# cuevhv/PMT_learning_for_semantic_segmentation_and_disparity

Measured on AMD Instinct MI355X. Metric: stereo-pairs/sec (train fwd+bwd) 512x256, higher is better.
Workload: dtype bf16; 1 GPU; minidsnetExt (densenet121, 1dcorr, aspp 0; the live PyTorch form of baseline_SDnet*) train step fwd+loss(CE+CE+Lovasz+L1)+bwd+Adam, 512x256 (WxH), batch 8 per GPU, hipGraph; global_batch=8, parallelism=dp1, world_size=1

## Files before the change

### include/sdhip.h

```cpp
#ifndef SDHIP_H_
#define SDHIP_H_

#include <stdint.h>

#ifdef __cplusplus
extern "C" {
#endif

#define SDHIP_F32 0
#define SDHIP_BF16 1

#define SDHIP_OK 0
#define SDHIP_ERR_ARG (-1)
#define SDHIP_ERR_LAUNCH (-2)
#define SDHIP_ERR_UNSUPPORTED (-3)

#define SDHIP_ACT_HSWISH 5
#define SDHIP_ACT_HSIGMOID 6

int sdhip_abi_version(void);
const char* sdhip_last_error(void);
void sdhip_diag_reload(void);
int sdhip_abort_capture(void* stream);
int sdhip_graph_node_counts(void* graph, int* counts);
// ... 12 lines not shown
int sdhip_conv_pack_weights(const float* src, void* dst, int M, int K, int T,
                            long stride_m, long stride_k, int flip, int dtype, void* stream);
int sdhip_conv_unpack_wgrad(const float* acc, float* grad, int M, int K, int T,
                            long stride_m, long stride_k, int flip, int accumulate, int dtype, void* stream);

int sdhip_conv2d_fwd(const void* x, const void* wpacked, void* y,
                     const float* bias, const float* in_scale, const float* in_shift,
                     double* stats, int stats_ld, int stats_nrep,
                     int B, int H, int W, int Cin, int ldx,
                     int Ho, int Wo, int Cout, int ldy,
                     int kh, int kw, int stride, int dil, int pad_t, int pad_l,
                     int D, int Do, int kd, int sd, int pad_d,
                     int in_relu, int groups, int act, int accumulate,
                     int dtype, void* stream);

int sdhip_conv2d_fwd_bnpro(const void* x, const void* wpacked, void* y, double* out_stats, int out_stats_ld, int out_stats_nrep,
                           double* in_stats, int in_stats_ld, int in_stats_nrep,
                           const double* pend_stats, int pend_ld, int pend_nrep, int pend_c0, int pend_n,
                           const float* gamma, const float* beta,
                           float* running_mean, float* running_var, float* scale_out, float* shift_out, float* mean_out,
                           float* invstd_out, double count, float eps, float momentum,
                           int B, int H, int W, int Cin, int ldx, int Ho, int Wo, int Cout, int ldy,
                           int kh, int kw, int pad_t, int pad_l, int groups, int dtype, void* stream);

int sdhip_conv2d_fwd_add(const void* x, const void* wpacked, void* y, const void* addend, int ldadd,
                         int B, int H, int W, int Cin, int ldx, int Ho, int Wo, int Cout, int ldy,
                         int kh, int kw, int pad_t, int pad_l, int dtype, void* stream);

int sdhip_conv2d_fwd_bnbwd(const void* x, const void* wpacked, void* y, double* sums, int sums_ld, int sums_nrep,
                           const void* u, int ldu, const float* scale, const float* shift, const void* addend, int ldadd,
                           int B, int H, int W, int Cin, int ldx, int Ho, int Wo, int Cout, int ldy,
                           int kh, int kw, int dil, int pad_t, int pad_l, int groups, int mode, int dtype, void* stream);

int sdhip_conv2d_fwd_phase(const void* x, const void* wpacked, void* y, double* stats, int stats_ld, int stats_nrep,
                           int B, int H, int W, int Cin, int ldx, int Cout, int ldy, int kh, int kw,
                           int D, int kd, int groups, int off_d, int off_h, int off_w, int dtype, void* stream);
int sdhip_conv2d_wgrad(const void* x, const void* dy, float* dw_packed, float* dbias,
                       const float* in_scale, const float* in_shift,
                       int B, int H, int W, int Cin, int ldx,
                       int Ho, int Wo, int Cout, int lddy,
                       int kh, int kw, int stride, int dil, int pad_t, int pad_l,
                       int D, int Do, int kd, int sd, int pad_d,
                       int in_relu, int groups, int prezeroed, int dtype, void* stream);
typedef struct SdhipWgradItem {
  const void* x; const void* dy; float* dw_packed; float* dbias; const float* in_scale; const float* in_shift;
  int B, H, W, Cin, ldx, Ho, Wo, Cout, lddy, kh, kw, stride, dil, pad_t, pad_l, D, Do, kd, sd, pad_d, in_relu, groups;
// ... 199 lines not shown
```

### pmt_learning_for_semantic_segmentation_and_disparity_amd/csrc/conv_fast.h

```cpp
#pragma once
#include "conv_common.h"

namespace {

struct FastArgs {
  const void* x; const void* wp; void* y;
  const float* bias; const float* in_scale; const float* in_shift; double* stats;
  int B, H, W, Ho, Wo, kh, kw, stride, dil, pad_t, pad_l;
  int D, Do, kd, sd, pad_d;
  int Cin, ldx, Cout, Mpad, ldy;
  int in_relu, bpg, act, accumulate;
  unsigned magic_iwp, magic_tw;
  int tiles_w, ntg;
  int tg, stats_ld, nrep, tail, dma;
  long rep_stride;
  int omul, ooz, ooy, oox;
  const void* bx; const float* bsc; const float* bsh; int ldbx;
  const void* res; int ldres;
  int bx_mode, bx_groups;
  const double* pin_stats; int pin_ld, pin_nrep, pin_groups, pin_off, pin_cs;
  const float* pin_gamma; const float* pin_beta;
  float* pin_scale; float* pin_shift; float* pin_mean; float* pin_invstd; float* pin_rmean; float* pin_rvar;
  float pin_eps, pin_momentum; double pin_count;
  const double* pend_stats; double* pin_fold; int pend_ld, pend_nrep, pend_c0, pend_n;
// ... 11 lines not shown
#pragma clang diagnostic pop
__device__ __forceinline__ unsigned lds_addr(const void* p) {
  return (unsigned)(size_t)(const __attribute__((address_space(3))) unsigned char*)p;
}

template <int CTRL> __device__ __forceinline__ float dpp_add(float v) {
  return v + __builtin_bit_cast(float, __builtin_amdgcn_update_dpp(0, __builtin_bit_cast(int, v), CTRL, 0xf, 0xf, true));
}
__device__ __forceinline__ float row16_sum(float v) {
  v = dpp_add<0xB1>(v);
  v = dpp_add<0x4E>(v);
  v = dpp_add<0x141>(v);
  return dpp_add<0x140>(v);
}

template <int KS> struct LdsRow;
template <> struct LdsRow<2> {
  static __device__ __forceinline__ int off(int row, int c) { return row * 128 + ((c ^ (row & 6)) << 4); }
};
template <> struct LdsRow<1> {
  static __device__ __forceinline__ int off(int row, int c) { return row * 64 + ((c ^ ((row >> 1) & 2)) << 4); }
};

template <typename T, int TH, int TW, int BN, int KS, bool DMA, bool BX = false>
__global__ __launch_bounds__(256) void conv_fast_kernel(const FastArgs p) {
  constexpr int V = Chunk<T>::N;
  constexpr int CK = 8 * V;
  constexpr int CKS = 4 * KS * V;
  constexpr int RB = 64 * KS;
  constexpr int SH = KS + 1;
  constexpr int CH = 4 * KS;
  constexpr int TWT = TW / 16, NPT = TH * TWT, NT_PIX = NPT / 4, NT_CO = BN / 16;
  constexpr bool PF = (TH * TW <= 64);
  constexpr int HPF = (DMA && KS == 1) ? 6 : 5;
  static_assert(NPT % 4 == 0 && NT_PIX >= 1, "every wave needs at least one 16-pixel MFMA tile");
  extern __shared__ __attribute__((aligned(16))) unsigned char smem[];

  const int tid = threadIdx.x, lane = tid & 63, wave = tid >> 6;
  const int l15 = lane & 15, lg = lane >> 4;
  const int s = p.stride, d = p.dil;
  const int tiles_w = p.tiles_w;
  const int ty = fast_div(blockIdx.x, tiles_w, p.magic_tw);
  const int oh0 = ty * TH, ow0 = (blockIdx.x - ty * tiles_w) * TW;
  const int n0 = blockIdx.y * BN;
  const int b = p.Do == 1 ? (int)blockIdx.z : (int)blockIdx.z / p.Do, dz = blockIdx.z - b * p.Do;
  const int grp = b < p.bpg ? 0 : b / p.bpg;
  const int IH = (TH - 1) * s + (p.kh - 1) * d + 1, IW = (TW - 1) * s + (p.kw - 1) * d + 1;
  const int IWp = (IW + 7) & ~7;
  const int ih0 = oh0 * s - p.pad_t, iw0 = ow0 * s - p.pad_l;
  const int Tn = p.kh * p.kw;
  const int nq = KS == 2 ? (p.Cin + CK - 1) / CK : 1;
  const int nqq = p.kd * nq;
  const int halo_bytes = ((IH * IWp + (256 >> SH) - 1) & ~((256 >> SH) - 1)) * RB;
  const int wbuf_bytes = ((p.tg * BN + (256 >> SH) - 1) & ~((256 >> SH) - 1)) * RB;
  unsigned char* const halo0 = smem;
  unsigned char* const wl0 = smem + halo_bytes * ((PF && nqq > 1) ? 2 : 1);

  f32x4 acc[NT_CO][NT_PIX];
#pragma unroll
  for (int mi = 0; mi < NT_CO; ++mi)
#pragma unroll
    for (int ni = 0; ni < NT_PIX; ++ni) acc[mi][ni] = f32x4{0.f, 0.f, 0.f, 0.f};

  const T* const xb0 = (const T*)p.x + (long)b * p.D * p.H * p.W * p.ldx;
  const T* const wpk = (const T*)p.wp;
  const int ntg = p.ntg;

  const int pt0 = wave * NT_PIX;
  const int prow0 = ((pt0 / TWT) * s) * IWp + ((pt0 % TWT) * 16 + l15) * s;
  int pdelta[NT_PIX];
#pragma unroll
  for (int ni = 0; ni < NT_PIX; ++ni) {
    const int pt = pt0 + ni;
    pdelta[ni] = (((pt / TWT) - (pt0 / TWT)) * s * IWp + ((pt % TWT) - (pt0 % TWT)) * 16 * s) * RB;
  }
  const int lg4 = lg << 4;
  const int a_base = LdsRow<KS>::off(l15, lg);

  constexpr int RPR = 256 >> SH;
  const int rsub = tid >> SH;
  const int c_l = (tid & (CH - 1)) ^ (KS == 2 ? (rsub & 6) : ((rsub >> 1) & 2));
  const int tid16 = tid * 16;
  const unsigned wave_lds = __builtin_amdgcn_readfirstlane(lds_addr(smem) + wave * 1024);
  const unsigned magic_iwp = p.magic_iwp;
  constexpr bool dma = DMA;
  float* const ptab_sc = reinterpret_cast<float*>(smem + (DMA ? 0 : p.pin_off));
  float* const ptab_sh = ptab_sc + (DMA ? 0 : p.pin_cs);
  const bool has_pro = p.in_scale != nullptr || (!DMA && p.pin_stats != nullptr);
  const int h_rows = IH * IWp;
  const int h_rounds = (h_rows + RPR - 1) / RPR;
  int h_src[HPF];
  if constexpr (PF) {
#pragma unroll
    for (int j = 0; j < HPF; ++j) {
      const int row = rsub + j * RPR;
      const int ih = fast_div(row, IWp, magic_iwp), iw = row - ih * IWp;
      const int gh = ih0 + ih, gw = iw0 + iw;
      h_src[j] = (row < h_rows && iw < IW && gh >= 0 && gh < p.H && gw >= 0 && gw < p.W) ? (gh * p.W + gw) * p.ldx + c_l * V : -1;
    }
  }
  const int mvalid = min(BN, p.Mpad - n0);

  u32x4 rh[HPF];
  const bool flat = p.kd == 1;
  auto chunk_of = [&](int qq) { return flat ? qq : qq % nq; };
  auto slice_of = [&](int qq) { return flat ? dz * p.sd - p.pad_d : dz * p.sd + qq / nq - p.pad_d; };

  auto mask_tail = [&](u32x4 raw, int ch0) -> u32x4 {
    const int nv = p.Cin - ch0;
    if (nv < V) {
      float f[V];
      Chunk<T>::unpack(raw, f);
#pragma unroll
      for (int e = 0; e < V; ++e) f[e] = e < nv ? f[e] : 0.f;
      raw = Chunk<T>::pack(f);
    }
    return raw;
  };
  float psc[V], psf[V];
  auto prologue_load = [&](int ch0) {
    if (ch0 < p.Cin) {
      if constexpr (!DMA) {
        if (p.pin_stats) {
#pragma unroll
          for (int e = 0; e < V; ++e) { psc[e] = ptab_sc[ch0 + e]; psf[e] = ptab_sh[ch0 + e]; }
          return;
// ... 28 lines not shown
#pragma unroll
    for (int j = 0; j < HPF; ++j) {
      if (j < h_rounds) {
        const T* src = (ok && h_src[j] >= 0) ? xb + h_src[j] : (const T*)sdhip_zero16;
        if constexpr (dma) glds16(src, (unsigned)(dst - smem) + j * 4096 + wave_lds);
        else rh[j] = *reinterpret_cast<const u32x4*>(src);
      }
    }
  };
  auto halo_commit = [&](int qq, unsigned char* dst) {
    const int ch0 = chunk_of(qq) * CKS + c_l * V;
    const int din = slice_of(qq);
    const bool ok = din >= 0 && din < p.D && ch0 < p.Cin;
    if (has_pro) prologue_load(ch0);
#pragma unroll
    for (int j = 0; j < HPF; ++j) {
      if (j < h_rounds) {
        u32x4 raw = rh[j];
        if (ok && h_src[j] >= 0) {
          if (p.tail) raw = mask_tail(raw, ch0);
          if (has_pro) raw = prologue(raw);
        }
        *reinterpret_cast<u32x4*>(dst + j * 4096 + tid16) = raw;
      }
    }
  };
  auto halo_sync_stage = [&](int qq, unsigned char* dst) {
    const int ch0 = chunk_of(qq) * CKS + c_l * V;
    const int din = slice_of(qq);
    const bool ok = din >= 0 && din < p.D && ch0 < p.Cin;
    const T* xb = xb0 + (long)din * p.H * p.W * p.ldx + ch0;
    auto src_of = [&](int j) -> const T* {
      const int row = rsub + j * RPR;
      const int ih = fast_div(row, IWp, magic_iwp), iw = row - ih * IWp;
      const int gh = ih0 + ih, gw = iw0 + iw;
      const bool in = ok && iw < IW && gh >= 0 && gh < p.H && gw >= 0 && gw < p.W;
      return in ? xb + (gh * p.W + gw) * p.ldx : (const T*)sdhip_zero16;
    };
    if constexpr (dma) {
      for (int j = 0; j < h_rounds; ++j) glds16(src_of(j), (unsigned)(dst - smem) + j * 4096 + wave_lds);
    } else {
      if (has_pro) prologue_load(ch0);
      for (int j0 = 0; j0 < h_rounds; j0 += 4) {
        u32x4 raw[4];
        bool in[4];
#pragma unroll
        for (int j = 0; j < 4; ++j) {
          if (j0 + j < h_rounds) {
            const T* src = src_of(j0 + j);
            in[j] = src != (const T*)sdhip_zero16;
            raw[j] = *reinterpret_cast<const u32x4*>(src);
          }
        }
#pragma unroll
        for (int j = 0; j < 4; ++j) {
          if (j0 + j < h_rounds) {
            if (in[j] && p.tail) raw[j] = mask_tail(raw[j], ch0);
            if (in[j] && has_pro) raw[j] = prologue(raw[j]);
            *reinterpret_cast<u32x4*>(dst + (j0 + j) * 4096 + tid16) = raw[j];
          }
        }
      }
    }
  };
  constexpr int RPT = BN >= RPR ? BN / RPR : 1;
  constexpr int TPR = BN >= RPR ? 1 : RPR / BN;
  auto w_issue = [&](int qq, int t0, unsigned char* dst) {
    const int nt = min(p.tg, Tn - t0);
    const T* base = wpk + ((long)(qq * Tn + t0) * p.Mpad + n0) * CK + c_l * V;
    unsigned lds = (unsigned)(dst - smem) + wave_lds;
    if constexpr (BN >= RPR) {
      for (int tl = 0; tl < nt; ++tl) {
#pragma unroll
        for (int r = 0; r < RPT; ++r) {
          const int m = min(r * RPR + rsub, mvalid - 1);
          glds16(base + (tl * p.Mpad + m) * CK, lds);
          lds += 4096;
        }
      }
    } else {
      const int m = min(rsub % BN, mvalid - 1);
      for (int t = 0; t < nt; t += TPR) {
        const int tl = min(t + rsub / BN, nt - 1);
        glds16(base + (tl * p.Mpad + m) * CK, lds);
        lds += 4096;
      }
    }
  };

  int kwi = 0, tap_off = 0;
  const int tap_row_step = d * IWp - p.kw * d;
  auto compute = [&](int t0, const unsigned char* halo, const unsigned char* wl) {
    const int nt = min(p.tg, Tn - t0);
    const int n = nt * KS;
    u32x4 af[2][NT_CO], bf[2][NT_PIX];
    int b_addr = 0, a_addr = 0;
    auto next_tap = [&](int tl) {
      const int row = prow0 + tap_off;
      if constexpr (KS == 2) b_addr = row * RB + (lg4 ^ ((row & 6) << 4));
      else b_addr = row * RB + (lg4 ^ (((row >> 1) & 2) << 4));
      a_addr = a_base + tl * (BN * RB);
      tap_off += d;
      if (++kwi == p.kw) { kwi = 0; tap_off += tap_row_step; }
    };
    auto load = [&](int set, int ks) {
      const unsigned char* ab = wl + (a_addr ^ (ks << 6));
      const unsigned char* bb = halo + (b_addr ^ (ks << 6));
#pragma unroll
      for (int mi = 0; mi < NT_CO; ++mi) af[set][mi] = *reinterpret_cast<const u32x4*>(ab + mi * (16 * RB));
#pragma unroll
      for (int ni = 0; ni < NT_PIX; ++ni) bf[set][ni] = *reinterpret_cast<const u32x4*>(bb + pdelta[ni]);
    };
    auto mma = [&](int set) {
#pragma unroll
      for (int mi = 0; mi < NT_CO; ++mi)
#pragma unroll
        for (int ni = 0; ni < NT_PIX; ++ni) Mma<T>::run(acc[mi][ni], af[set][mi], bf[set][ni]);
    };
    if constexpr (KS == 2) {
      next_tap(0);
      load(0, 0);
      for (int tl = 0; tl < nt; ++tl) {
        load(1, 1);
        mma(0);
        if (tl + 1 < nt) { next_tap(tl + 1); load(0, 0); }
        mma(1);
      }
    } else {
      next_tap(0);
      load(0, 0);
      for (int u = 0; u < n; u += 2) {
        if (u + 1 < n) { next_tap(u + 1); load(1, 0); }
        mma(0);
        if (u + 2 < n) { next_tap(u + 2); load(0, 0); }
        if (u + 1 < n) mma(1);
      }
    }
  };

  w_issue(0, 0, wl0);
  if constexpr (PF) halo_issue(0, halo0);
  if constexpr (!DMA) {
    if (p.pin_stats) {
      const int G = p.pin_groups;
      auto sums_of = [&](int g, int c, double& a1, double& a2) {
        a1 = 0.; a2 = 0.;
        const int cp = c - p.pend_c0;
        if (cp >= 0 && cp < p.pend_n) {
          for (int r = 0; r < p.pend_nrep; ++r) {
            const double* Sr = p.pend_stats + (long)r * G * 2 * p.pend_ld;
            a1 += Sr[((long)g * 2 + 0) * p.pend_ld + cp];
            a2 += Sr[((long)g * 2 + 1) * p.pend_ld + cp];
          }
        } else {
          for (int r = 0; r < p.pin_nrep; ++r) {
            const double* Sr = p.pin_stats + (long)r * G * 2 * p.pin_ld;
            a1 += Sr[((long)g * 2 + 0) * p.pin_ld + c];
            a2 += Sr[((long)g * 2 + 1) * p.pin_ld + c];
          }
        }
      };
      for (int c = tid; c < p.Cin; c += 256) {
        double a1, a2;
        sums_of(grp, c, a1, a2);
        const double mu = a1 / p.pin_count;
        double var = a2 / p.pin_count - mu * mu;
// ... 11 lines not shown
          for (int g = 0; g < G; ++g) {
            double a1, a2;
            sums_of(g, c, a1, a2);
            if (pend) {
              p.pin_fold[((long)g * 2 + 0) * p.pin_ld + c] = a1;
              p.pin_fold[((long)g * 2 + 1) * p.pin_ld + c] = a2;
            }
            const double mu = a1 / p.pin_count;
            double var = a2 / p.pin_count - mu * mu;
            if (var < 0.) var = 0.;
            const float inv = (float)(1.0 / sqrt(var + (double)p.pin_eps));
            const float scv = gm * inv;
            p.pin_scale[g * p.Cin + c] = scv;
            p.pin_shift[g * p.Cin + c] = (float)((double)bt - mu * (double)scv);
            p.pin_mean[g * p.Cin + c] = (float)mu;
            p.pin_invstd[g * p.Cin + c] = inv;
            const double unb = p.pin_count > 1. ? var * p.pin_count / (p.pin_count - 1.) : var;
            rm = (1.f - p.pin_momentum) * rm + p.pin_momentum * (float)mu;
            rv = (1.f - p.pin_momentum) * rv + p.pin_momentum * (float)unb;
          }
          if (p.pin_rmean) { p.pin_rmean[c] = rm; p.pin_rvar[c] = rv; }
        }
      }
      __syncthreads();
    }
  }
  if constexpr (!PF) halo_sync_stage(0, halo0);
  int q = 0, tgi = 0;
  const int S = nqq * ntg;
  for (int st = 0; st < S; ++st) {
    const int t0 = tgi * p.tg;
    unsigned char* halo = halo0 + ((PF && (q & 1)) ? halo_bytes : 0);
    unsigned char* wl = wl0 + (st & 1) * wbuf_bytes;
    if constexpr (PF && !dma) { if (tgi == 0) halo_commit(q, halo); }
    asm volatile("s_waitcnt vmcnt(0)" ::: "memory");
    __syncthreads();
    int qn = q, tgn = tgi + 1;
    if (tgn == ntg) { tgn = 0; ++qn; }
    const bool more = st + 1 < S;
    if (more) {
      if (PF && tgn == 0) halo_issue(qn, halo0 + ((qn & 1) ? halo_bytes : 0));
      w_issue(qn, tgn * p.tg, wl0 + ((st + 1) & 1) * wbuf_bytes);
    }
    compute(t0, halo, wl);
    if (!PF && more && tgn == 0) {
      asm volatile("s_waitcnt vmcnt(0)" ::: "memory");
      __syncthreads();
      halo_sync_stage(qn, halo0);
    }
    if (tgn == 0) { kwi = 0; tap_off = 0; }
    q = qn; tgi = tgn;
  }
// ... 180 lines not shown
        if (l15 == 0) {
          const int m = mi * 16 + 4 * lg + r;
          red[(wave * 2 + 0) * BN + m] = a;
          red[(wave * 2 + 1) * BN + m] = c2;
        }
      }
    }
    __syncthreads();
    if (tid < 2 * BN) {
      const int which = tid / BN, m = tid - which * BN;
      if (n0 + m < p.Cout) {
        const float tot = red[(0 * 2 + which) * BN + m] + red[(1 * 2 + which) * BN + m] +
                          red[(2 * 2 + which) * BN + m] + red[(3 * 2 + which) * BN + m];
        const long rep = (blockIdx.x + blockIdx.z) % p.nrep;
        if (BX && p.bx_mode == 1)
          atomicAdd(reinterpret_cast<float*>(p.stats) + (((long)which * p.nrep + rep) * p.bx_groups + grp) * p.Cout + n0 + m, tot);
        else
          atomicAdd(p.stats + rep * p.rep_stride + ((long)grp * 2 + which) * p.stats_ld + n0 + m, (double)tot);
      }
    }
  }
}

template <typename T, int TH, int TW, int BN, int KS, bool DMA, bool BX = false>
int launch_fast(const FastArgs& a, size_t lds, hipStream_t s) {
  auto kern = conv_fast_kernel<T, TH, TW, BN, KS, DMA, BX>;
  static bool attr_set = false;
  if (lds > 64 * 1024 && !attr_set) {
    if (hipFuncSetAttribute((const void*)kern, hipFuncAttributeMaxDynamicSharedMemorySize, 160 * 1024) != hipSuccess)
      SDHIP_FAIL(SDHIP_ERR_LAUNCH, "conv_fast: cannot raise dynamic LDS limit");
    attr_set = true;
  }
  dim3 grid(sdhip_cdiv(a.Ho, TH) * sdhip_cdiv(a.Wo, TW), sdhip_cdiv(a.Mpad, BN), a.B * a.Do);
  hipLaunchKernelGGL(kern, grid, dim3(256), lds, s, a);
  SDHIP_LAUNCH_CHECK();
  return SDHIP_OK;
}

template <typename T, int TH, int TW, int KS, bool DMA>
int launch_fast_bn(const FastArgs& a, int bn, size_t lds, hipStream_t s) {
  switch (bn) {
    case 16: return launch_fast<T, TH, TW, 16, KS, DMA>(a, lds, s);
    case 32: return launch_fast<T, TH, TW, 32, KS, DMA>(a, lds, s);
    case 64: return launch_fast<T, TH, TW, 64, KS, DMA>(a, lds, s);
    default: return launch_fast<T, TH, TW, 128, KS, DMA>(a, lds, s);
  }
}

template <typename T, bool DMA>
int launch_fast_tile(const FastArgs& a, bool big, int ks, int bn, size_t lds, hipStream_t s) {
  if (big) return ks == 2 ? launch_fast_bn<T, 8, 32, 2, DMA>(a, bn, lds, s) : launch_fast_bn<T, 8, 32, 1, DMA>(a, bn, lds, s);
  return ks == 2 ? launch_fast_bn<T, 4, 16, 2, DMA>(a, bn, lds, s) : launch_fast_bn<T, 4, 16, 1, DMA>(a, bn, lds, s);
}

template <int TH, int TW, int KS>
int launch_fast_bx_bn(const FastArgs& a, int bn, size_t lds, hipStream_t s) {
  switch (bn) {
    case 16: return launch_fast<bf16_t, TH, TW, 16, KS, true, true>(a, lds, s);
    case 32: return launch_fast<bf16_t, TH, TW, 32, KS, true, true>(a, lds, s);
    case 64: return launch_fast<bf16_t, TH, TW, 64, KS, true, true>(a, lds, s);
    default: return launch_fast<bf16_t, TH, TW, 128, KS, true, true>(a, lds, s);
  }
}

template <typename T>
int launch_fast_any(const FastArgs& a, bool big, int ks, int bn, size_t lds, hipStream_t s) {
  if (a.bx) {
    if (!a.dma || sizeof(T) != 2) SDHIP_FAIL(SDHIP_ERR_UNSUPPORTED, "conv2d_fwd_bnbwd: bf16 without an input prologue / channel tail only");
    if (big) return ks == 2 ? launch_fast_bx_bn<8, 32, 2>(a, bn, lds, s) : launch_fast_bx_bn<8, 32, 1>(a, bn, lds, s);
    return ks == 2 ? launch_fast_bx_bn<4, 16, 2>(a, bn, lds, s) : launch_fast_bx_bn<4, 16, 1>(a, bn, lds, s);
  }
  return a.dma ? launch_fast_tile<T, true>(a, big, ks, bn, lds, s) : launch_fast_tile<T, false>(a, big, ks, bn, lds, s);
}

}
```

### pmt_learning_for_semantic_segmentation_and_disparity_amd/csrc/conv_fwd.hip

```cpp
#include "conv_common.h"
#include "conv_fast.h"
#include "conv_band.h"
#include "conv_gemm.h"
#include "conv_thin.h"

namespace {

struct FwdArgs {
  const void* x; const void* wp; void* y;
  const float* bias; const float* in_scale; const float* in_shift; double* stats;
  ConvGeom g;
  int Cin, ldx, Cout, Mpad, ldy;
  int in_relu, groups, act, accumulate;
  int tg, vec_in, vec_out, stats_ld, nrep, pf_halo, sh, per_tap;
  long rep_stride;
};

template <typename T, int TH, int TW, int BN>
__global__ __launch_bounds__(256) void conv_fwd_kernel(const FwdArgs p) {
  constexpr int V = Chunk<T>::N;
  constexpr int CK = 8 * V;
  constexpr int TWT = TW / 16;
  constexpr int NPT = TH * TWT;
  constexpr int NT_PIX = NPT / 4;
// ... 338 lines not shown
  hipLaunchKernelGGL(kern, grid, dim3(256), lds, s, a);
  SDHIP_LAUNCH_CHECK();
  return SDHIP_OK;
}

template <typename T, int TH, int TW>
int launch_bn(const FwdArgs& a, int bn, size_t lds, hipStream_t s) {
  switch (bn) {
    case 16: return launch<T, TH, TW, 16>(a, lds, s);
    case 32: return launch<T, TH, TW, 32>(a, lds, s);
    case 64: return launch<T, TH, TW, 64>(a, lds, s);
    default: return launch<T, TH, TW, 128>(a, lds, s);
  }
}

size_t halo_bytes_of(const ConvGeom& g, int th, int tw, int per_tap) {
  const int eh = per_tap ? 0 : (g.kh - 1) * g.dil, ew = per_tap ? 0 : (g.kw - 1) * g.dil;
  const int IH = (th - 1) * g.stride + eh + 1, IW = (tw - 1) * g.stride + ew + 1;
  return ((size_t)IH * IW * 128 + 15) & ~(size_t)15;
}

}

struct ProStats {
  const double* stats; int ld, nrep;
  const float* gamma; const float* beta;
  float* scale; float* shift; float* mean; float* invstd; float* rmean; float* rvar;
  float eps, momentum; double count;
  const double* pend; double* fold; int pend_ld, pend_nrep, pend_c0, pend_n;
};

static int conv2d_fwd_impl(const void* x, const void* wpacked, void* y,
                           const float* bias, const float* in_scale, const float* in_shift,
                           double* stats, int stats_ld, int stats_nrep,
                           int B, int H, int W, int Cin, int ldx,
                           int Ho, int Wo, int Cout, int ldy,
                           int kh, int kw, int stride, int dil, int pad_t, int pad_l,
                           int D, int Do, int kd, int sd, int pad_d,
                           int in_relu, int groups, int act, int accumulate,
                           int dtype, void* stream, int omul, int ooz, int ooy, int oox,
                           const void* bx = nullptr, int ldbx = 0, const float* bsc = nullptr, const float* bsh = nullptr,
                           const void* addend = nullptr, int ldadd = 0, int bx_mode = 0, const ProStats* ps = nullptr) {
  SDHIP_CHECK_ARG(x && wpacked && y, "conv2d_fwd: null pointer");
  SDHIP_CHECK_ARG(dtype == SDHIP_F32 || dtype == SDHIP_BF16, "conv2d_fwd: unknown dtype %d", dtype);
  SDHIP_CHECK_ARG(B > 0 && H > 0 && W > 0 && Cin > 0 && Cout > 0 && Ho > 0 && Wo > 0, "conv2d_fwd: empty tensor");
  SDHIP_CHECK_ARG(ldx >= Cin && ldy >= Cout, "conv2d_fwd: pixel stride smaller than channel count");
  SDHIP_CHECK_ARG(kh >= 1 && kw >= 1 && stride >= 1 && dil >= 1, "conv2d_fwd: bad kernel geometry");
  SDHIP_CHECK_ARG(groups >= 1 && B % groups == 0, "conv2d_fwd: batch %d not divisible by %d stat groups", B, groups);
  SDHIP_CHECK_ARG((in_scale == nullptr) == (in_shift == nullptr), "conv2d_fwd: in_scale/in_shift must come together");
  SDHIP_CHECK_ARG(((uintptr_t)wpacked & 15) == 0, "conv2d_fwd: packed weights must be 16-byte aligned");
  const int V = dtype == SDHIP_BF16 ? 8 : 4;
  const int es = conv_esize(dtype);
  FwdArgs a;
  a.x = x; a.wp = wpacked; a.y = y; a.bias = bias; a.in_scale = in_scale; a.in_shift = in_shift; a.stats = stats;
  SDHIP_CHECK_ARG(D >= 1 && Do >= 1 && kd >= 1 && sd >= 1 && (long)B * Do <= 65535, "conv2d_fwd: bad depth geometry");
  a.g = ConvGeom{B, H, W, Ho, Wo, kh, kw, stride, dil, pad_t, pad_l, D, Do, kd, sd, pad_d};
  a.Cin = Cin; a.ldx = ldx; a.Cout = Cout; a.Mpad = (Cout + 15) & ~15; a.ldy = ldy;
  a.in_relu = in_relu; a.groups = groups; a.act = act; a.accumulate = accumulate;
  a.stats_ld = stats_ld > 0 ? stats_ld : Cout;
  a.nrep = stats_nrep > 0 ? stats_nrep : 1;
  a.rep_stride = (long)groups * 2 * a.stats_ld;
  a.vec_in = (ldx % V == 0) && (((uintptr_t)x & 15) == 0);
  a.vec_out = (ldy % 4 == 0) && (((uintptr_t)y % (4 * es)) == 0);
  int bn = 16;
  for (int cand = 128; cand >= 32; cand >>= 1)
    if ((long)sdhip_cdiv(a.Mpad, cand) * cand * 4 <= (long)a.Mpad * 5) { bn = cand; break; }
  if ((long)kh * kw * kd * Cin <= 128 && a.Mpad <= 128) bn = a.Mpad > 64 ? 128 : (a.Mpad > 32 ? 64 : (a.Mpad > 16 ? 32 : 16));
  const int T = kh * kw;
  const long blocks_big = (long)sdhip_cdiv(Ho, 8) * sdhip_cdiv(Wo, 32) * B * Do * sdhip_cdiv(a.Mpad, bn);
  const SdhipDiag& dg = sdhip_diag();
  const int tune_big = dg.tune_big, tune_split = dg.tune_split;
  const int tune_ksoft_small = 80, tune_ksoft_big = 80;
  bool big = (blocks_big >= tune_big && Wo >= 24) || dg.conv_big;
  if (stride == 2 && kd > 1 && !dg.conv_big && dg.tune_s2_small) big = false;
  if (!big) {
// ... 92 lines not shown
    f.Cin = Cin; f.ldx = ldx; f.Cout = Cout; f.Mpad = a.Mpad; f.ldy = ldy;
    f.in_relu = in_relu; f.bpg = B / groups; f.act = act; f.accumulate = accumulate;
    f.stats_ld = a.stats_ld; f.nrep = a.nrep; f.rep_stride = a.rep_stride; f.tail = (Cin % V) != 0;
    f.omul = omul; f.ooz = ooz; f.ooy = ooy; f.oox = oox;
    f.bx = bx; f.ldbx = ldbx; f.bsc = bsc; f.bsh = bsh;
    f.res = bx ? addend : nullptr; f.ldres = ldadd; f.bx_mode = bx_mode; f.bx_groups = groups;
    f.dma = !in_scale && !f.tail && !ps;
    f.pin_stats = nullptr;
    if (ps) {
      f.pin_stats = ps->stats; f.pin_ld = ps->ld; f.pin_nrep = ps->nrep; f.pin_groups = groups; f.pin_gamma = ps->gamma; f.pin_beta = ps->beta;
      f.pin_scale = ps->scale; f.pin_shift = ps->shift; f.pin_mean = ps->mean; f.pin_invstd = ps->invstd; f.pin_rmean = ps->rmean; f.pin_rvar = ps->rvar;
      f.pin_eps = ps->eps; f.pin_momentum = ps->momentum; f.pin_count = ps->count;
      f.pend_stats = ps->pend; f.pin_fold = ps->fold; f.pend_ld = ps->pend_ld; f.pend_nrep = ps->pend_nrep; f.pend_c0 = ps->pend_c0; f.pend_n = ps->pend ? ps->pend_n : 0;
    }
    bool fbig = big;
    for (int attempt = 0; attempt < 2; ++attempt) {
      const int th = fbig ? 8 : 4, tw = fbig ? 32 : 16;
      const int IH = (th - 1) * stride + (kh - 1) * dil + 1, IW = (tw - 1) * stride + (kw - 1) * dil + 1;
      const int IWp = (IW + 7) & ~7;
      const int hrows = ((IH * IWp + px_per_round - 1) / px_per_round) * px_per_round;
      const int nqq_f = kd * (ks == 2 ? sdhip_cdiv(Cin, CKh) : 1);
      const size_t hb = (size_t)hrows * rb * ((fbig || nqq_f == 1) ? 1 : 2);
      if (!fbig && hrows > ((f.dma && ks == 1) ? 6 : 5) * px_per_round) { fbig = true; continue; }
      auto wbuf = [&](int tgv) { return (size_t)(((tgv * bn + px_per_round - 1) / px_per_round) * px_per_round) * rb; };
      int tg = T;
      const size_t ksoft_f = (size_t)(fbig ? tune_ksoft_big : tune_ksoft_small) * 1024;
      size_t lds;
      if (nqq_f == 1 && hb + wbuf(T) <= ksoft_f) {
        lds = hb + wbuf(T);
      } else {
        while (tg > 1 && hb + 2 * wbuf(tg) > ksoft_f) --tg;
        lds = hb + 2 * wbuf(tg);
      }
      if (lds < 4096) lds = 4096;
      f.pin_off = 0; f.pin_cs = 0;
      if (ps) { f.pin_off = (int)lds; f.pin_cs = (Cin + 63) & ~63; lds += 2 * (size_t)f.pin_cs * sizeof(float); }
      if (lds > kMax) { if (!fbig) break; fbig = false; continue; }
      f.tg = tg;
      f.magic_iwp = IWp > 1 ? (unsigned)(0x100000000ULL / (unsigned)IWp) + 1u : 0u;
      f.tiles_w = sdhip_cdiv(Wo, tw);
      f.magic_tw = f.tiles_w > 1 ? (unsigned)(0x100000000ULL / (unsigned)f.tiles_w) + 1u : 0u;
      f.ntg = sdhip_cdiv(T, tg);
      if ((long)f.tiles_w * sdhip_cdiv(Ho, th) >= 65536) break;
      return dtype == SDHIP_BF16 ? launch_fast_any<bf16_t>(f, fbig, ks, bn, lds, s) : launch_fast_any<float>(f, fbig, ks, bn, lds, s);
    }
  }
  if (omul != 1) SDHIP_FAIL(SDHIP_ERR_UNSUPPORTED, "conv2d_fwd_phase: interleaved output needs the aligned fast path (ldx %% 8, ldy %% 4)");
  if (ps) SDHIP_FAIL(SDHIP_ERR_UNSUPPORTED, "conv2d_fwd_bnpro: needs the aligned fast path (ldx %% 8, ldy %% 4, halo tile within LDS)");
  if (bx) SDHIP_FAIL(SDHIP_ERR_UNSUPPORTED, "conv2d_fwd_bnbwd: needs the aligned fast path (ldx %% 8, ldy %% 4, halo tile within LDS)");
  for (int attempt = 0; attempt < 2; ++attempt) {
    const int th = big ? 8 : 4, tw = big ? 32 : 16;
    const int per_tap = per_tap_any;
    const size_t halo = halo_bytes_of(a.g, th, tw, per_tap);
    const long halo_loads = (long)(halo / 128) * chunks_per_row;
    const int pf = !per_tap && !big && a.vec_in && (Cin % V == 0) && halo_loads <= 4 * 256 && 2 * halo + 2 * (size_t)bn * 128 <= kSoft;
    int tg = per_tap ? 1 : 1024 / (rows * chunks_per_row);
    if (tg < 1) tg = 1;
    if (tg > T) tg = T;
    const size_t hb = halo * (pf ? 2 : 1);
    while (tg > 1 && hb + 2 * (size_t)tg * bn * 128 > kSoft) --tg;
    size_t lds = hb + 2 * (size_t)tg * bn * 128;
    if (lds < 4096) lds = 4096;
    if (lds > kMax) {
      if (big) { big = false; continue; }
      SDHIP_FAIL(SDHIP_ERR_UNSUPPORTED, "conv2d_fwd: halo tile of a %dx%d kernel with dilation %d does not fit LDS", kh, kw, dil);
    }
// ... 93 lines not shown
```

### pmt_learning_for_semantic_segmentation_and_disparity_amd/csrc/runtime.hip

```cpp
#include "sdhip_common.h"
#include <vector>

#define SDHIP_ABI_VERSION 2

static thread_local char g_err[512] = "";

void sdhip_set_error(const char* fmt, ...) {
  va_list ap;
  va_start(ap, fmt);
  vsnprintf(g_err, sizeof(g_err), fmt, ap);
  va_end(ap);
}

extern "C" int sdhip_abi_version(void) { return SDHIP_ABI_VERSION; }
extern "C" const char* sdhip_last_error(void) { return g_err; }

static SdhipDiag g_diag;
static bool g_diag_init = false;

static int env_int(const char* name, int dflt) { const char* v = getenv(name); return v ? atoi(v) : dflt; }
static bool env_set(const char* name) {
  const char* v = getenv(name);
  if (v && *v) { fprintf(stderr, "[libsdhip] diagnostic switch %s=%s is set: kernels / launch heuristics differ from production\n", name, v); return true; }
  return false;
}
static void diag_fill() {
  g_diag.conv_generic = env_set("SDHIP_CONV_GENERIC");
  g_diag.conv_big = env_set("SDHIP_CONV_BIG");
  g_diag.conv_no_thin = env_set("SDHIP_CONV_NO_THIN");
  g_diag.conv_no_gemm = env_set("SDHIP_CONV_NO_GEMM");
  g_diag.conv_no_band = env_set("SDHIP_CONV_NO_BAND");
  g_diag.conv_no_band3 = env_set("SDHIP_CONV_NO_BAND3");
  g_diag.wgrad_generic = env_set("SDHIP_WGRAD_GENERIC");
  g_diag.wgrad_no_pack = env_set("SDHIP_WGRAD_NO_PACK");
  g_diag.wgrad_force_pack = env_set("SDHIP_WGRAD_FORCE_PACK");
  g_diag.wgrad_no_half = env_set("SDHIP_WGRAD_NO_HALF");
  g_diag.thin_wgrad_reg = env_set("SDHIP_THIN_WGRAD_REG");
  g_diag.corr_no_tiled = env_set("SDHIP_CORR_NO_TILED");
  g_diag.wgrad_no_half32 = env_set("SDHIP_WGRAD_NO_HALF32");
  g_diag.wgrad_split2d = env_set("SDHIP_WGRAD_SPLIT2D");
  g_diag.tune_s2_small = env_int("SDHIP_TUNE_S2_SMALL", 1);
  g_diag.tune_big = env_int("SDHIP_TUNE_BIG", 512);
  g_diag.tune_split = env_int("SDHIP_TUNE_SPLIT", 1024);
  g_diag.tune_thin_blocks = env_int("SDHIP_TUNE_THIN_BLOCKS", 1024);
  g_diag.tune_fused_blocks = env_int("SDHIP_TUNE_FUSED_BLOCKS", 768);
  g_diag.tune_gemm_dbg = env_int("SDHIP_TUNE_GEMM_DBG", 0);
  g_diag.tune_band_dbg = env_int("SDHIP_TUNE_BAND_DBG", 0);
  g_diag.tune_atomic_tbs = getenv("SDHIP_TUNE_ATOMIC_TBS") ? atof(getenv("SDHIP_TUNE_ATOMIC_TBS")) : 1.3;
  g_diag_init = true;
}
const SdhipDiag& sdhip_diag() {
  if (!g_diag_init) diag_fill();
  return g_diag;
}
__attribute__((constructor)) static void diag_at_load() { diag_fill(); }
extern "C" void sdhip_diag_reload(void) { diag_fill(); }

extern "C" int sdhip_abort_capture(void* stream) {
  hipStream_t s = (hipStream_t)stream;
  hipStreamCaptureStatus st = hipStreamCaptureStatusNone;
  hipError_t e = hipStreamIsCapturing(s, &st);
  (void)hipGetLastError();
  int was_open = 0;
  if (e != hipSuccess || st != hipStreamCaptureStatusNone) {
    hipGraph_t g = nullptr;
    (void)hipStreamEndCapture(s, &g);
    (void)hipGetLastError();
    if (g) (void)hipGraphDestroy(g);
    was_open = 1;
  }
// ... 25 lines not shown
```

### pmt_learning_for_semantic_segmentation_and_disparity_amd/csrc/sdhip_common.h

```cpp
#pragma once
#include <hip/hip_runtime.h>
#include <stdint.h>
#include <stdio.h>
#include <stdarg.h>
#include <stdlib.h>

#include "../../include/sdhip.h"

#define SDHIP_WAVE 64

typedef unsigned short bf16_t;

typedef __attribute__((ext_vector_type(4))) float f32x4;
typedef __attribute__((ext_vector_type(2))) float f32x2;
typedef __attribute__((ext_vector_type(8))) __bf16 bf16x8_t;
typedef __attribute__((ext_vector_type(4))) __bf16 bf16x4_t;
typedef __attribute__((ext_vector_type(4))) unsigned int u32x4;
typedef __attribute__((ext_vector_type(2))) unsigned int u32x2;

void sdhip_set_error(const char* fmt, ...);
#define SDHIP_FAIL(code, ...) do { sdhip_set_error(__VA_ARGS__); return (code); } while (0)
#define SDHIP_CHECK_ARG(cond, ...) do { if (!(cond)) SDHIP_FAIL(SDHIP_ERR_ARG, __VA_ARGS__); } while (0)
#define SDHIP_LAUNCH_CHECK() do { hipError_t e__ = hipGetLastError(); \
    if (e__ != hipSuccess) SDHIP_FAIL(SDHIP_ERR_LAUNCH, "%s: launch failed: %s", __func__, hipGetErrorString(e__)); } while (0)

struct SdhipDiag {
  bool conv_generic, conv_big, conv_no_thin, conv_no_gemm, conv_no_band, conv_no_band3, wgrad_generic, wgrad_no_pack, wgrad_force_pack, wgrad_no_half, thin_wgrad_reg, corr_no_tiled, wgrad_no_half32, wgrad_split2d;
  int tune_s2_small;
  int tune_big, tune_split, tune_thin_blocks, tune_fused_blocks, tune_gemm_dbg, tune_band_dbg;
  double tune_atomic_tbs;
};
const SdhipDiag& sdhip_diag();

__device__ __forceinline__ float bf2f(bf16_t v) { return __builtin_bit_cast(float, ((unsigned int)v) << 16); }
__device__ __forceinline__ bf16_t f2bf(float f) { return __builtin_bit_cast(bf16_t, (__bf16)f); }
__device__ __forceinline__ unsigned int pack2bf(float lo, float hi) {
  return (unsigned int)f2bf(lo) | ((unsigned int)f2bf(hi) << 16);
}
__device__ __forceinline__ float bflo(unsigned int u) { return __builtin_bit_cast(float, u << 16); }
__device__ __forceinline__ float bfhi(unsigned int u) { return __builtin_bit_cast(float, u & 0xffff0000u); }

template <typename T> struct Elem;
template <> struct Elem<float> {
  static constexpr int kPer16B = 4;
  static __device__ __forceinline__ float ld(const float* p) { return *p; }
  static __device__ __forceinline__ void st(float* p, float v) { *p = v; }
  static __device__ __forceinline__ float rnd(float v) { return v; }
};
template <> struct Elem<bf16_t> {
  static constexpr int kPer16B = 8;
  static __device__ __forceinline__ float ld(const bf16_t* p) { return bf2f(*p); }
  static __device__ __forceinline__ void st(bf16_t* p, float v) { *p = f2bf(v); }
// ... 88 lines not shown
```

Baseline: 382.4 stereo-pairs/s.

## Add deep-K conv path staging multiple channel chunks per double-buffered stage

```diff
diff --git a/include/sdhip.h b/include/sdhip.h
--- a/include/sdhip.h
+++ b/include/sdhip.h
@@ -58,6 +58,7 @@
                            float* invstd_out, double count, float eps, float momentum,
                            int B, int H, int W, int Cin, int ldx, int Ho, int Wo, int Cout, int ldy,
                            int kh, int kw, int pad_t, int pad_l, int groups, int dtype, void* stream);
+int sdhip_conv_last_plan(int* plan);
 
 int sdhip_conv2d_fwd_add(const void* x, const void* wpacked, void* y, const void* addend, int ldadd,
                          int B, int H, int W, int Cin, int ldx, int Ho, int Wo, int Cout, int ldy,
diff --git a/pmt_learning_for_semantic_segmentation_and_disparity_amd/csrc/conv_fast.h b/pmt_learning_for_semantic_segmentation_and_disparity_amd/csrc/conv_fast.h
--- a/pmt_learning_for_semantic_segmentation_and_disparity_amd/csrc/conv_fast.h
+++ b/pmt_learning_for_semantic_segmentation_and_disparity_amd/csrc/conv_fast.h
@@ -57,7 +57,10 @@
   static __device__ __forceinline__ int off(int row, int c) { return row * 64 + ((c ^ ((row >> 1) & 2)) << 4); }
 };
 
-template <typename T, int TH, int TW, int BN, int KS, bool DMA, bool BX = false>
+constexpr int kDeepK = 4;
+constexpr int kDeepKRows = 64;
+
+template <typename T, int TH, int TW, int BN, int KS, bool DMA, bool BX = false, bool DK = false>
 __global__ __launch_bounds__(256) void conv_fast_kernel(const FastArgs p) {
   constexpr int V = Chunk<T>::N;
   constexpr int CK = 8 * V;
@@ -69,6 +72,8 @@
   constexpr bool PF = (TH * TW <= 64);
   constexpr int HPF = (DMA && KS == 1) ? 6 : 5;
   static_assert(NPT % 4 == 0 && NT_PIX >= 1, "every wave needs at least one 16-pixel MFMA tile");
+  static_assert(!DK || (PF && !DMA && !BX && KS == 2 && TH * TW == kDeepKRows), "deep K: register-staging 4x16 form, 128-byte rows");
+  constexpr int NRH = DK ? 2 * kDeepK : HPF;
   extern __shared__ __attribute__((aligned(16))) unsigned char smem[];
 
   const int tid = threadIdx.x, lane = tid & 63, wave = tid >> 6;
@@ -89,7 +94,9 @@
   const int halo_bytes = ((IH * IWp + (256 >> SH) - 1) & ~((256 >> SH) - 1)) * RB;
   const int wbuf_bytes = ((p.tg * BN + (256 >> SH) - 1) & ~((256 >> SH) - 1)) * RB;
   unsigned char* const halo0 = smem;
-  unsigned char* const wl0 = smem + halo_bytes * ((PF && nqq > 1) ? 2 : 1);
+  const int gk = DK ? p.tg : 1;
+  const int hstage_bytes = halo_bytes * gk;
+  unsigned char* const wl0 = smem + (DK ? 2 * hstage_bytes : halo_bytes * ((PF && nqq > 1) ? 2 : 1));
 
   f32x4 acc[NT_CO][NT_PIX];
 #pragma unroll
@@ -136,7 +143,7 @@
   }
   const int mvalid = min(BN, p.Mpad - n0);
 
-  u32x4 rh[HPF];
+  u32x4 rh[NRH];
   const bool flat = p.kd == 1;
   auto chunk_of = [&](int qq) { return flat ? qq : qq % nq; };
   auto slice_of = [&](int qq) { return flat ? dz * p.sd - p.pad_d : dz * p.sd + qq / nq - p.pad_d; };
@@ -211,6 +218,39 @@
           if (has_pro) raw = prologue(raw);
         }
         *reinterpret_cast<u32x4*>(dst + j * 4096 + tid16) = raw;
+      }
+    }
+  };
+  auto halo_issue_dk = [&](int q0, int nt) {
+#pragma unroll
+    for (int c = 0; c < kDeepK; ++c) {
+      if (c < nt) {
+        const bool ok = (q0 + c) * CKS + c_l * V < p.Cin;
+        const T* xb = xb0 + (q0 + c) * CKS;
+#pragma unroll
+        for (int j = 0; j < 2; ++j) {
+          const T* src = (ok && h_src[j] >= 0) ? xb + h_src[j] : (const T*)sdhip_zero16;
+          rh[c * 2 + j] = *reinterpret_cast<const u32x4*>(src);
+        }
+      }
+    }
+  };
+  auto halo_commit_dk = [&](int q0, int nt, unsigned char* dst) {
+#pragma unroll
+    for (int c = 0; c < kDeepK; ++c) {
+      if (c < nt) {
+        const int ch0 = (q0 + c) * CKS + c_l * V;
+        const bool ok = ch0 < p.Cin;
+        if (has_pro) prologue_load(ch0);
+#pragma unroll
+        for (int j = 0; j < 2; ++j) {
+          u32x4 raw = rh[c * 2 + j];
+          if (ok && h_src[j] >= 0) {
+            if (p.tail) raw = mask_tail(raw, ch0);
+            if (has_pro) raw = prologue(raw);
+          }
+          *reinterpret_cast<u32x4*>(dst + c * (kDeepKRows * RB) + j * 4096 + tid16) = raw;
+        }
       }
     }
   };
@@ -255,7 +295,7 @@
   constexpr int RPT = BN >= RPR ? BN / RPR : 1;
   constexpr int TPR = BN >= RPR ? 1 : RPR / BN;
   auto w_issue = [&](int qq, int t0, unsigned char* dst) {
-    const int nt = min(p.tg, Tn - t0);
+    const int nt = DK ? min(p.tg, nq - qq) : min(p.tg, Tn - t0);
     const T* base = wpk + ((long)(qq * Tn + t0) * p.Mpad + n0) * CK + c_l * V;
     unsigned lds = (unsigned)(dst - smem) + wave_lds;
     if constexpr (BN >= RPR) {
@@ -280,7 +320,7 @@
   int kwi = 0, tap_off = 0;
   const int tap_row_step = d * IWp - p.kw * d;
   auto compute = [&](int t0, const unsigned char* halo, const unsigned char* wl) {
-    const int nt = min(p.tg, Tn - t0);
+    const int nt = DK ? min(p.tg, nq - t0) : min(p.tg, Tn - t0);
     const int n = nt * KS;
     u32x4 af[2][NT_CO], bf[2][NT_PIX];
     int b_addr = 0, a_addr = 0;
@@ -289,8 +329,12 @@
       if constexpr (KS == 2) b_addr = row * RB + (lg4 ^ ((row & 6) << 4));
       else b_addr = row * RB + (lg4 ^ (((row >> 1) & 2) << 4));
       a_addr = a_base + tl * (BN * RB);
+      if constexpr (DK) {
+        tap_off += kDeepKRows;
+      } else {
       tap_off += d;
       if (++kwi == p.kw) { kwi = 0; tap_off += tap_row_step; }
+      }
     };
     auto load = [&](int set, int ks) {
       const unsigned char* ab = wl + (a_addr ^ (ks << 6));
@@ -328,9 +372,106 @@
   };
 
   w_issue(0, 0, wl0);
-  if constexpr (PF) halo_issue(0, halo0);
+  if constexpr (DK) halo_issue_dk(0, min(gk, nq));
+  else if constexpr (PF) halo_issue(0, halo0);
   if constexpr (!DMA) {
     if (p.pin_stats) {
+      if constexpr (DK) {
+      const int G = p.pin_groups;
+      constexpr int PC = kPinMaxC / 256;
+      const int nrmax = max(p.pin_nrep, p.pend_n ? p.pend_nrep : 0);
+      auto sums_pc = [&](int g, double (&a1)[PC], double (&a2)[PC]) {
+        const double* src[PC];
+        long rs[PC];
+        int sq[PC], nr[PC];
+        bool live[PC];
+#pragma unroll
+        for (int i = 0; i < PC; ++i) {
+          const int c0 = tid + i * 256;
+          live[i] = c0 < p.Cin;
+          const int c = live[i] ? c0 : 0;
+          const int cp = c - p.pend_c0;
+          if (cp >= 0 && cp < p.pend_n) {
+            src[i] = p.pend_stats + ((long)g * 2 + 0) * p.pend_ld + cp; sq[i] = p.pend_ld; rs[i] = (long)G * 2 * p.pend_ld; nr[i] = p.pend_nrep;
+          } else {
+            src[i] = p.pin_stats + ((long)g * 2 + 0) * p.pin_ld + c; sq[i] = p.pin_ld; rs[i] = (long)G * 2 * p.pin_ld; nr[i] = p.pin_nrep;
+          }
+          a1[i] = 0.; a2[i] = 0.;
+        }
+        for (int r = 0; r < nrmax; ++r) {
+          double v1[PC], v2[PC];
+#pragma unroll
+          for (int i = 0; i < PC; ++i) {
+            const double* Sr = src[i] + min(r, nr[i] - 1) * rs[i];
+            v1[i] = Sr[0]; v2[i] = Sr[sq[i]];
+          }
+#pragma unroll
+          for (int i = 0; i < PC; ++i) {
+            if (live[i] && r < nr[i]) { a1[i] += v1[i]; a2[i] += v2[i]; }
+          }
+        }
+      };
+      {
+        double a1[PC], a2[PC];
+        sums_pc(grp, a1, a2);
+#pragma unroll
+        for (int i = 0; i < PC; ++i) {
+          const int c = tid + i * 256;
+          if (c < p.Cin) {
+            const double mu = a1[i] / p.pin_count;
+            double var = a2[i] / p.pin_count - mu * mu;
+            if (var < 0.) var = 0.;
+            const float inv = (float)(1.0 / sqrt(var + (double)p.pin_eps));
+            const float scv = (p.pin_gamma ? p.pin_gamma[c] : 1.f) * inv;
+            ptab_sc[c] = scv;
+            ptab_sh[c] = (float)((double)(p.pin_beta ? p.pin_beta[c] : 0.f) - mu * (double)scv);
+          }
+        }
+      }
+      if (blockIdx.x == 0 && blockIdx.y == 0 && blockIdx.z == 0) {
+        float gm[PC], bt[PC], rm[PC], rv[PC];
+#pragma unroll
+        for (int i = 0; i < PC; ++i) {
+          const int c = tid + i * 256;
+          const bool ok = c < p.Cin;
+          gm[i] = ok && p.pin_gamma ? p.pin_gamma[c] : 1.f; bt[i] = ok && p.pin_beta ? p.pin_beta[c] : 0.f;
+          rm[i] = ok && p.pin_rmean ? p.pin_rmean[c] : 0.f; rv[i] = ok && p.pin_rvar ? p.pin_rvar[c] : 0.f;
+        }
+        for (int g = 0; g < G; ++g) {
+          double a1[PC], a2[PC];
+          sums_pc(g, a1, a2);
+#pragma unroll
+          for (int i = 0; i < PC; ++i) {
+            const int c = tid + i * 256;
+            if (c < p.Cin) {
+              if (c >= p.pend_c0 && c < p.pend_c0 + p.pend_n) {
+                p.pin_fold[((long)g * 2 + 0) * p.pin_ld + c] = a1[i];
+                p.pin_fold[((long)g * 2 + 1) * p.pin_ld + c] = a2[i];
+              }
+              const double mu = a1[i] / p.pin_count;
+              double var = a2[i] / p.pin_count - mu * mu;
+              if (var < 0.) var = 0.;
+              const float inv = (float)(1.0 / sqrt(var + (double)p.pin_eps));
+              const float scv = gm[i] * inv;
+              p.pin_scale[g * p.Cin + c] = scv;
+              p.pin_shift[g * p.Cin + c] = (float)((double)bt[i] - mu * (double)scv);
+              p.pin_mean[g * p.Cin + c] = (float)mu;
+              p.pin_invstd[g * p.Cin + c] = inv;
+              const double unb = p.pin_count > 1. ? var * p.pin_count / (p.pin_count - 1.) : var;
+              rm[i] = fmaf(1.f - p.pin_momentum, rm[i], p.pin_momentum * (float)mu);
+              rv[i] = fmaf(1.f - p.pin_momentum, rv[i], p.pin_momentum * (float)unb);
+            }
+          }
+        }
+        if (p.pin_rmean) {
+#pragma unroll
+          for (int i = 0; i < PC; ++i) {
+            const int c = tid + i * 256;
+            if (c < p.Cin) { p.pin_rmean[c] = rm[i]; p.pin_rvar[c] = rv[i]; }
+          }
+        }
+      }
+      } else {
       const int G = p.pin_groups;
       auto sums_of = [&](int g, int c, double& a1, double& a2) {
         a1 = 0.; a2 = 0.;
@@ -388,12 +529,30 @@
           if (p.pin_rmean) { p.pin_rmean[c] = rm; p.pin_rvar[c] = rv; }
         }
       }
+      }
       __syncthreads();
+    }
+  }
+  if constexpr (DK) {
+    const int S = (nq + gk - 1) / gk;
+    for (int st = 0; st < S; ++st) {
+      const int q0 = st * gk;
+      unsigned char* halo = halo0 + (st & 1) * hstage_bytes;
+      unsigned char* wl = wl0 + (st & 1) * wbuf_bytes;
+      halo_commit_dk(q0, min(gk, nq - q0), halo);
+      asm volatile("s_waitcnt vmcnt(0)" ::: "memory");
+      __syncthreads();
+      if (st + 1 < S) {
+        halo_issue_dk(q0 + gk, min(gk, nq - q0 - gk));
+        w_issue(q0 + gk, 0, wl0 + ((st + 1) & 1) * wbuf_bytes);
+      }
+      compute(q0, halo, wl);
+      tap_off = 0;
     }
   }
   if constexpr (!PF) halo_sync_stage(0, halo0);
   int q = 0, tgi = 0;
-  const int S = nqq * ntg;
+  const int S = DK ? 0 : nqq * ntg;
   for (int st = 0; st < S; ++st) {
     const int t0 = tgi * p.tg;
     unsigned char* halo = halo0 + ((PF && (q & 1)) ? halo_bytes : 0);
@@ -620,9 +779,9 @@
   }
 }
 
-template <typename T, int TH, int TW, int BN, int KS, bool DMA, bool BX = false>
+template <typename T, int TH, int TW, int BN, int KS, bool DMA, bool BX = false, bool DK = false>
 int launch_fast(const FastArgs& a, size_t lds, hipStream_t s) {
-  auto kern = conv_fast_kernel<T, TH, TW, BN, KS, DMA, BX>;
+  auto kern = conv_fast_kernel<T, TH, TW, BN, KS, DMA, BX, DK>;
   static bool attr_set = false;
   if (lds > 64 * 1024 && !attr_set) {
     if (hipFuncSetAttribute((const void*)kern, hipFuncAttributeMaxDynamicSharedMemorySize, 160 * 1024) != hipSuccess)
@@ -662,7 +821,18 @@
 }
 
 template <typename T>
-int launch_fast_any(const FastArgs& a, bool big, int ks, int bn, size_t lds, hipStream_t s) {
+int launch_fast_dk(const FastArgs& a, int bn, size_t lds, hipStream_t s) {
+  switch (bn) {
+    case 16: return launch_fast<T, 4, 16, 16, 2, false, false, true>(a, lds, s);
+    case 32: return launch_fast<T, 4, 16, 32, 2, false, false, true>(a, lds, s);
+    case 64: return launch_fast<T, 4, 16, 64, 2, false, false, true>(a, lds, s);
+    default: return launch_fast<T, 4, 16, 128, 2, false, false, true>(a, lds, s);
+  }
+}
+
+template <typename T>
+int launch_fast_any(const FastArgs& a, bool big, int ks, int bn, size_t lds, hipStream_t s, bool deepk = false) {
+  if (deepk) return launch_fast_dk<T>(a, bn, lds, s);
   if (a.bx) {
     if (!a.dma || sizeof(T) != 2) SDHIP_FAIL(SDHIP_ERR_UNSUPPORTED, "conv2d_fwd_bnbwd: bf16 without an input prologue / channel tail only");
     if (big) return ks == 2 ? launch_fast_bx_bn<8, 32, 2>(a, bn, lds, s) : launch_fast_bx_bn<8, 32, 1>(a, bn, lds, s);
diff --git a/pmt_learning_for_semantic_segmentation_and_disparity_amd/csrc/conv_fwd.hip b/pmt_learning_for_semantic_segmentation_and_disparity_amd/csrc/conv_fwd.hip
--- a/pmt_learning_for_semantic_segmentation_and_disparity_amd/csrc/conv_fwd.hip
+++ b/pmt_learning_for_semantic_segmentation_and_disparity_amd/csrc/conv_fwd.hip
@@ -384,6 +384,15 @@
 
 }
 
+static void deepk_pick(int nq, long px_blocks, int Mpad, int bn, int force_g, int force_bn, int* g, int* bnq) {
+  const long wgs = px_blocks * sdhip_cdiv(Mpad, bn);
+  *bnq = bn;
+  *g = wgs <= 256 ? kDeepK : (wgs <= 512 ? 3 : 0);
+  if (force_bn == 16 || force_bn == 32 || force_bn == 64 || force_bn == 128) *bnq = force_bn;
+  if (force_g >= 1 && force_g <= kDeepK) *g = force_g;
+  if (*g > nq) *g = nq;
+}
+
 struct ProStats {
   const double* stats; int ld, nrep;
   const float* gamma; const float* beta;
@@ -391,6 +400,14 @@
   float eps, momentum; double count;
   const double* pend; double* fold; int pend_ld, pend_nrep, pend_c0, pend_n;
 };
+
+static thread_local int g_last_plan[3] = {0, 0, 0};
+
+extern "C" int sdhip_conv_last_plan(int* plan) {
+  SDHIP_CHECK_ARG(plan, "conv_last_plan: null pointer");
+  for (int i = 0; i < 3; ++i) plan[i] = g_last_plan[i];
+  return SDHIP_OK;
+}
 
 static int conv2d_fwd_impl(const void* x, const void* wpacked, void* y,
                            const float* bias, const float* in_scale, const float* in_shift,
@@ -413,6 +430,7 @@
   SDHIP_CHECK_ARG(((uintptr_t)wpacked & 15) == 0, "conv2d_fwd: packed weights must be 16-byte aligned");
   const int V = dtype == SDHIP_BF16 ? 8 : 4;
   const int es = conv_esize(dtype);
+  g_last_plan[0] = g_last_plan[1] = g_last_plan[2] = 0;
   FwdArgs a;
   a.x = x; a.wp = wpacked; a.y = y; a.bias = bias; a.in_scale = in_scale; a.in_shift = in_shift; a.stats = stats;
   SDHIP_CHECK_ARG(D >= 1 && Do >= 1 && kd >= 1 && sd >= 1 && (long)B * Do <= 65535, "conv2d_fwd: bad depth geometry");
@@ -551,6 +569,28 @@
       const int nqq_f = kd * (ks == 2 ? sdhip_cdiv(Cin, CKh) : 1);
       const size_t hb = (size_t)hrows * rb * ((fbig || nqq_f == 1) ? 1 : 2);
       if (!fbig && hrows > ((f.dma && ks == 1) ? 6 : 5) * px_per_round) { fbig = true; continue; }
+      if (!fbig && !f.dma && !bx && T == 1 && kd == 1 && stride == 1 && D == 1 && Do == 1 && ks == 2 && Cin > 64 && hrows == kDeepKRows &&
+          !dg.conv_no_deepk) {
+        const long px_blocks = (long)sdhip_cdiv(Ho, 4) * sdhip_cdiv(Wo, 16) * B;
+        int gq, bnq;
+        deepk_pick(nqq_f, px_blocks, a.Mpad, bn, dg.tune_deepk_g, dg.tune_deepk_bn, &gq, &bnq);
+        auto wb = [&](int g) { return (size_t)(((g * bnq + px_per_round - 1) / px_per_round) * px_per_round) * rb; };
+        const size_t tab = ps ? 2 * (size_t)((Cin + 63) & ~63) * sizeof(float) : 0;
+        while (gq > 1 && 2 * (size_t)gq * kDeepKRows * rb + 2 * wb(gq) + tab > kMax) --gq;
+        size_t lds = 2 * (size_t)gq * kDeepKRows * rb + 2 * wb(gq);
+        if (gq >= 2 && lds + tab <= kMax) {
+          f.pin_off = 0; f.pin_cs = 0;
+          if (ps) { f.pin_off = (int)lds; f.pin_cs = (Cin + 63) & ~63; lds += tab; }
+          f.tg = gq; f.ntg = 1;
+          f.magic_iwp = (unsigned)(0x100000000ULL / 16u) + 1u;
+          f.tiles_w = sdhip_cdiv(Wo, tw);
+          f.magic_tw = f.tiles_w > 1 ? (unsigned)(0x100000000ULL / (unsigned)f.tiles_w) + 1u : 0u;
+          if ((long)f.tiles_w * sdhip_cdiv(Ho, th) < 65536) {
+            g_last_plan[0] = gq; g_last_plan[1] = bnq; g_last_plan[2] = 0;
+            return dtype == SDHIP_BF16 ? launch_fast_any<bf16_t>(f, false, ks, bnq, lds, s, true) : launch_fast_any<float>(f, false, ks, bnq, lds, s, true);
+          }
+        }
+      }
       auto wbuf = [&](int tgv) { return (size_t)(((tgv * bn + px_per_round - 1) / px_per_round) * px_per_round) * rb; };
       int tg = T;
       const size_t ksoft_f = (size_t)(fbig ? tune_ksoft_big : tune_ksoft_small) * 1024;
@@ -571,6 +611,7 @@
       f.magic_tw = f.tiles_w > 1 ? (unsigned)(0x100000000ULL / (unsigned)f.tiles_w) + 1u : 0u;
       f.ntg = sdhip_cdiv(T, tg);
       if ((long)f.tiles_w * sdhip_cdiv(Ho, th) >= 65536) break;
+      g_last_plan[1] = bn; g_last_plan[2] = fbig;
       return dtype == SDHIP_BF16 ? launch_fast_any<bf16_t>(f, fbig, ks, bn, lds, s) : launch_fast_any<float>(f, fbig, ks, bn, lds, s);
     }
   }
diff --git a/pmt_learning_for_semantic_segmentation_and_disparity_amd/csrc/runtime.hip b/pmt_learning_for_semantic_segmentation_and_disparity_amd/csrc/runtime.hip
--- a/pmt_learning_for_semantic_segmentation_and_disparity_amd/csrc/runtime.hip
+++ b/pmt_learning_for_semantic_segmentation_and_disparity_amd/csrc/runtime.hip
@@ -31,6 +31,7 @@
   g_diag.conv_no_gemm = env_set("SDHIP_CONV_NO_GEMM");
   g_diag.conv_no_band = env_set("SDHIP_CONV_NO_BAND");
   g_diag.conv_no_band3 = env_set("SDHIP_CONV_NO_BAND3");
+  g_diag.conv_no_deepk = env_set("SDHIP_CONV_NO_DEEPK");
   g_diag.wgrad_generic = env_set("SDHIP_WGRAD_GENERIC");
   g_diag.wgrad_no_pack = env_set("SDHIP_WGRAD_NO_PACK");
   g_diag.wgrad_force_pack = env_set("SDHIP_WGRAD_FORCE_PACK");
@@ -46,6 +47,8 @@
   g_diag.tune_fused_blocks = env_int("SDHIP_TUNE_FUSED_BLOCKS", 768);
   g_diag.tune_gemm_dbg = env_int("SDHIP_TUNE_GEMM_DBG", 0);
   g_diag.tune_band_dbg = env_int("SDHIP_TUNE_BAND_DBG", 0);
+  g_diag.tune_deepk_g = env_int("SDHIP_TUNE_DEEPK_G", 0);
+  g_diag.tune_deepk_bn = env_int("SDHIP_TUNE_DEEPK_BN", 0);
   g_diag.tune_atomic_tbs = getenv("SDHIP_TUNE_ATOMIC_TBS") ? atof(getenv("SDHIP_TUNE_ATOMIC_TBS")) : 1.3;
   g_diag_init = true;
 }
diff --git a/pmt_learning_for_semantic_segmentation_and_disparity_amd/csrc/sdhip_common.h b/pmt_learning_for_semantic_segmentation_and_disparity_amd/csrc/sdhip_common.h
--- a/pmt_learning_for_semantic_segmentation_and_disparity_amd/csrc/sdhip_common.h
+++ b/pmt_learning_for_semantic_segmentation_and_disparity_amd/csrc/sdhip_common.h
@@ -25,9 +25,9 @@
     if (e__ != hipSuccess) SDHIP_FAIL(SDHIP_ERR_LAUNCH, "%s: launch failed: %s", __func__, hipGetErrorString(e__)); } while (0)
 
 struct SdhipDiag {
-  bool conv_generic, conv_big, conv_no_thin, conv_no_gemm, conv_no_band, conv_no_band3, wgrad_generic, wgrad_no_pack, wgrad_force_pack, wgrad_no_half, thin_wgrad_reg, corr_no_tiled, wgrad_no_half32, wgrad_split2d;
+  bool conv_generic, conv_big, conv_no_thin, conv_no_gemm, conv_no_band, conv_no_band3, wgrad_generic, wgrad_no_pack, wgrad_force_pack, wgrad_no_half, thin_wgrad_reg, corr_no_tiled, wgrad_no_half32, wgrad_split2d, conv_no_deepk;
   int tune_s2_small;
-  int tune_big, tune_split, tune_thin_blocks, tune_fused_blocks, tune_gemm_dbg, tune_band_dbg;
+  int tune_big, tune_split, tune_thin_blocks, tune_fused_blocks, tune_gemm_dbg, tune_band_dbg, tune_deepk_g, tune_deepk_bn;
   double tune_atomic_tbs;
 };
 const SdhipDiag& sdhip_diag();
```

New measurement: 385.1 stereo-pairs/s (median of 6 runs). About the same (+0.7%).
